# voidstrike/FPSG

Hardware: AMD Instinct MI355X
Metric: episodes/sec (+ Chamfer-kernel HBM GB/s in roofline.hbm), 2048-pt clouds, 224x224 images; episode = fwd + Chamfer + bwd, step = E episodes + all-reduce + Adam (higher is better)
Workload: dtype f32

## Files before the change

### fpsg_amd/_hip.py

```python
from __future__ import annotations

import ctypes
import os
import threading

import torch

_HERE = os.path.dirname(os.path.abspath(__file__))
LIB_PATH = os.environ.get("FPSG_HIP_LIB") or os.path.join(_HERE, "libfpsg_hip.so")

_c_f32p = ctypes.c_void_p
_c_i32p = ctypes.c_void_p
_c_int = ctypes.c_int
_c_stream = ctypes.c_void_p

SIGNATURES = {
    "fpsg_version": [],
    "fpsg_last_error": [],
    "fpsg_chamfer_fwd": [_c_f32p, _c_f32p, _c_int, _c_int, _c_int,
                         _c_f32p, _c_i32p, _c_f32p, _c_i32p, _c_stream],
    "fpsg_chamfer_bwd": [_c_f32p, _c_f32p, _c_i32p, _c_i32p, _c_f32p, _c_f32p,
                         _c_int, _c_int, _c_int, _c_f32p, _c_f32p, _c_stream],
    "fpsg_chamfer_losses": [_c_f32p, _c_f32p, _c_int, _c_int, _c_int, _c_int, ctypes.c_float, ctypes.c_float, _c_f32p,
                            _c_stream],
# ... 62 lines not shown
    "fpsg_bn_act_rows_bwd": [_c_f32p, _c_int, ctypes.POINTER(ctypes.c_int), ctypes.POINTER(ctypes.c_int), _c_int,
                             _c_f32p, _c_f32p, _c_f32p, _c_int, _c_int, ctypes.c_float, _c_f32p, _c_f32p, _c_f32p,
                             _c_f32p, _c_stream],
    "fpsg_bn_workspace_floats": [_c_int, _c_int, _c_int],
    "fpsg_bn_act_fwd": [_c_f32p, _c_f32p, _c_f32p, _c_f32p, _c_f32p, _c_f32p, ctypes.c_float, _c_int, _c_int, _c_int, _c_int,
                        ctypes.c_float, _c_int, ctypes.c_float, _c_f32p, _c_f32p, _c_f32p, _c_f32p, _c_f32p,
                        _c_stream],
    "fpsg_bn_act_bwd": [_c_f32p, _c_f32p, _c_f32p, _c_f32p, _c_int, _c_int, _c_int, _c_int, _c_int,
                        ctypes.c_float, _c_f32p, _c_f32p, _c_f32p, _c_f32p, _c_f32p, _c_f32p, _c_stream],
    "fpsg_bn_act_bwd_coef": [_c_f32p, _c_f32p, _c_f32p, _c_f32p, _c_int, _c_int, _c_int, _c_int, _c_int, ctypes.c_float,
                             _c_f32p, _c_f32p, _c_f32p, _c_f32p, _c_stream],
    "fpsg_bn_act_bwd_parts": [_c_f32p, _c_f32p, _c_f32p, _c_f32p, _c_int, _c_int, _c_int, _c_int, _c_int,
                        ctypes.c_float, _c_f32p, _c_f32p, _c_f32p, _c_f32p, _c_f32p, _c_f32p, _c_f32p, _c_int, _c_stream],
    "fpsg_bn_pool_workspace_floats": [_c_int, _c_int, _c_int, _c_int],
    "fpsg_bn_act_pool_fwd": [_c_f32p, _c_f32p, _c_f32p, _c_f32p, _c_f32p, _c_f32p, ctypes.c_float, _c_int, _c_int, _c_int, _c_int,
                             _c_int, ctypes.c_float, _c_int, ctypes.c_float, _c_f32p, _c_f32p, _c_f32p, _c_f32p,
                             _c_f32p, _c_f32p, _c_int, _c_stream],
    "fpsg_bn_act_pool_bwd": [_c_f32p, _c_f32p, _c_f32p, _c_f32p, _c_int, _c_int, _c_int, _c_int, _c_int, _c_int,
                             ctypes.c_float, _c_f32p, _c_f32p, _c_f32p, _c_f32p, _c_f32p, _c_f32p, _c_stream],
    "fpsg_bn_max_workspace_floats": [_c_int, _c_int, _c_int],
    "fpsg_bn_max_dz_offset": [_c_int, _c_int, _c_int],
    "fpsg_bn_act_max_fwd": [_c_f32p, _c_f32p, _c_f32p, _c_f32p, _c_f32p, _c_f32p, ctypes.c_float, _c_int, _c_int, _c_int, _c_int,
                            ctypes.c_float, _c_int, ctypes.c_float, _c_f32p, _c_i32p, _c_f32p, _c_f32p, _c_f32p,
                            _c_f32p, _c_stream],
    "fpsg_bn_act_max_bwd": [_c_f32p, _c_f32p, _c_f32p, _c_i32p, _c_f32p, _c_int, _c_int, _c_int, _c_int, _c_int,
                            ctypes.c_float, _c_f32p, _c_f32p, _c_f32p, _c_f32p, _c_f32p, _c_f32p, _c_stream],
    "fpsg_max_bwd_prep": [_c_f32p, _c_f32p, _c_f32p, _c_f32p, _c_f32p, _c_f32p, _c_int, _c_int, _c_int, _c_int, _c_f32p, _c_f32p,
                          _c_f32p, _c_f32p, _c_stream],
    "fpsg_max_bwd_dw": [_c_f32p, _c_f32p, _c_f32p, _c_f32p, _c_f32p, _c_int, _c_int, _c_int, _c_f32p, _c_stream],
    "fpsg_max_bwd_gather": [_c_f32p, _c_f32p, _c_i32p, _c_int, _c_int, _c_int, _c_int, _c_f32p, _c_f32p, _c_stream],
    "fpsg_max_bwd_scatter": [_c_f32p, _c_f32p, _c_f32p, _c_f32p, _c_i32p, _c_f32p, _c_int, _c_int, _c_int, _c_int, _c_f32p,
                             _c_stream],
    "fpsg_max_bwd_scatter_workspace_floats": [_c_int, _c_int, _c_int],
    "fpsg_bn_act_max_bwd_coef": [_c_f32p, _c_f32p, _c_f32p, _c_i32p, _c_f32p, _c_int, _c_int, _c_int, _c_int, _c_int,
                                 ctypes.c_float, _c_f32p, _c_f32p, _c_f32p, _c_f32p, _c_stream],
    "fpsg_wino_input_transform": [_c_int, _c_f32p, _c_int, _c_int, _c_int, _c_int, _c_f32p, ctypes.c_long, _c_stream],
    "fpsg_wino_output_transform": [_c_int, _c_f32p, _c_int, _c_int, _c_int, _c_int, _c_f32p, ctypes.c_long, _c_stream],
    "fpsg_wino_stats_parts": [_c_int, _c_int, _c_int, _c_int],
    "fpsg_wino_output_transform_stats": [_c_int, _c_f32p, _c_int, _c_int, _c_int, _c_int, _c_f32p, _c_f32p, _c_f32p,
                                         ctypes.c_long, _c_stream],
    "fpsg_wino_grad_output_transform": [_c_int, _c_f32p, _c_int, _c_int, _c_int, _c_int, _c_f32p, ctypes.c_long, _c_stream],
    "fpsg_wino_grad_transforms": [_c_int, _c_f32p, _c_int, _c_int, _c_int, _c_int, _c_f32p, _c_f32p, ctypes.c_long, _c_stream],
    "fpsg_wino_filter_transform": [_c_int, _c_f32p, _c_int, _c_int, _c_int, _c_f32p, _c_stream],
    "fpsg_wino_output_transform_bwd_stats": [_c_int, _c_f32p, _c_int, _c_int, _c_int, _c_int, _c_f32p, _c_f32p, _c_f32p,
                                             _c_f32p, _c_f32p, ctypes.c_long, _c_stream],
    "fpsg_wino_filter_transform_batch": [ctypes.c_void_p, _c_int, ctypes.c_long, _c_stream],
    "fpsg_wino_filter_grad_transform": [_c_int, _c_f32p, _c_int, _c_int, _c_f32p, _c_stream],
    "fpsg_wino_conv_fused": [_c_f32p, _c_f32p, _c_int, _c_int, _c_int, _c_int, _c_int, _c_f32p, _c_stream],
    "fpsg_wino_input_transform_act": [_c_int, _c_f32p, _c_f32p, _c_f32p, _c_int, _c_int, _c_int, _c_int, _c_f32p, ctypes.c_long,
                                      _c_stream],
    "fpsg_wino_conv_fused_act": [_c_f32p, _c_f32p, _c_f32p, _c_f32p, _c_int, _c_int, _c_int, _c_int, _c_int, _c_f32p,
                                 _c_stream],
    "fpsg_wino_dw_fused_workspace_floats": [_c_int, _c_int, _c_int, _c_int],
    "fpsg_wino_dw_fused": [_c_f32p, _c_f32p, _c_f32p, _c_f32p, _c_int, _c_int, _c_int, _c_int, _c_int, _c_f32p, _c_f32p,
                           _c_stream],
    "fpsg_wino_conv_fused_parts": [_c_int, _c_int, _c_int, _c_int],
    "fpsg_wino_conv_fused_stats": [_c_f32p, _c_f32p, _c_f32p, _c_f32p, _c_int, _c_int, _c_int, _c_int, _c_int, _c_f32p,
                                   _c_f32p, _c_f32p, _c_stream],
    "fpsg_bn_stats": [_c_f32p, _c_f32p, _c_f32p, _c_f32p, _c_f32p, _c_f32p, ctypes.c_float, _c_int, _c_int, _c_int, _c_int,
                      ctypes.c_float, _c_f32p, _c_f32p, _c_f32p, _c_f32p, _c_f32p, _c_int, _c_stream],
    "fpsg_conv_first_dw_workspace_floats": [_c_int, _c_int, _c_int],
    "fpsg_conv_first_parts": [_c_int, _c_int, _c_int],
    "fpsg_conv_first_fwd": [_c_f32p, _c_f32p, _c_int, _c_int, _c_int, _c_int, _c_int, _c_f32p, _c_f32p, _c_f32p, _c_stream],
    "fpsg_conv_first_dw": [_c_f32p, _c_f32p, _c_int, _c_int, _c_int, _c_int, _c_int, _c_f32p, _c_f32p, _c_stream],
    "fpsg_conv_first_dw_fold": [_c_f32p, _c_f32p, _c_f32p, _c_f32p, _c_f32p, _c_f32p, _c_int, _c_int, _c_int, _c_int, _c_int,
                                _c_f32p, _c_f32p, _c_stream],
# ... 96 lines not shown
    "fpsg_points_render": [_c_f32p, ctypes.c_void_p, _c_int, _c_int, _c_f32p, _c_int, _c_int, _c_int, _c_int,
                           ctypes.c_float, ctypes.c_float, ctypes.POINTER(ctypes.c_float), _c_int, ctypes.c_void_p,
                           ctypes.c_void_p, _c_f32p, _c_i32p, _c_f32p, ctypes.c_void_p, ctypes.c_size_t, _c_stream],
    "fpsg_episode_views": [ctypes.c_void_p, _c_int, _c_int, _c_int, _c_i32p, _c_int, _c_i32p, _c_f32p, _c_f32p, _c_int,
                           _c_int, _c_stream],
    "fpsg_point_mesh_workspace_bytes": [_c_int, _c_int, _c_int, _c_int],
    "fpsg_point_mesh_distance": [_c_f32p, _c_int, _c_int, _c_f32p, _c_int, _c_int, _c_i32p, _c_int, _c_int, _c_f32p,
                                 _c_i32p, _c_f32p, _c_f32p, ctypes.c_void_p, ctypes.c_size_t, _c_stream],
    "fpsg_point_normals_workspace_bytes": [_c_int, _c_int, _c_int],
    "fpsg_point_normals": [_c_f32p, _c_int, _c_int, _c_int, _c_int, _c_f32p, _c_f32p, _c_f32p, _c_i32p, ctypes.c_void_p,
                           ctypes.c_size_t, _c_stream],
    "fpsg_point_normals_orient_workspace_bytes": [_c_int, _c_int, _c_int],
    "fpsg_point_normals_orient": [_c_f32p, _c_f32p, _c_i32p, _c_int, _c_int, _c_int, _c_int, _c_f32p, _c_i32p,
                                  ctypes.c_void_p, ctypes.c_size_t, _c_stream],
}
_RESTYPES = {"fpsg_last_error": ctypes.c_char_p, "fpsg_grad_norm_workspace_bytes": ctypes.c_size_t,
"fpsg_chamfer_workspace_bytes": ctypes.c_size_t,
             "fpsg_sinkhorn_workspace_floats": ctypes.c_size_t,
             "fpsg_sinkhorn_grad_workspace_floats": ctypes.c_size_t,
             "fpsg_knn_workspace_floats": ctypes.c_size_t,
             "fpsg_bn_workspace_floats": ctypes.c_size_t, "fpsg_bn_pool_workspace_floats": ctypes.c_size_t, "fpsg_bn_max_workspace_floats": ctypes.c_size_t, "fpsg_bn_max_dz_offset": ctypes.c_size_t, "fpsg_conv_first_dw_workspace_floats": ctypes.c_size_t, "fpsg_emd_workspace_floats": ctypes.c_size_t, "fpsg_emd_exact_workspace_floats": ctypes.c_size_t, "fpsg_emd_cross_workspace_bytes": ctypes.c_size_t, "fpsg_occupancy_grid_workspace_bytes": ctypes.c_size_t, "fpsg_fps_workspace_bytes": ctypes.c_size_t, "fpsg_max_bwd_scatter_workspace_floats": ctypes.c_size_t,
             "fpsg_wino_dw_fused_workspace_floats": ctypes.c_size_t, "fpsg_gemm_split_workspace_floats": ctypes.c_size_t, "fpsg_gemm_split_packed_a_bytes": ctypes.c_size_t, "fpsg_edgeconv_stats_ws_floats": ctypes.c_size_t,
             "fpsg_repulsion_workspace_bytes": ctypes.c_size_t,
             "fpsg_expansion_workspace_bytes": ctypes.c_size_t,
             "fpsg_uniform_workspace_bytes": ctypes.c_size_t,
             "fpsg_swd_workspace_bytes": ctypes.c_size_t,
             "fpsg_mesh_cdf_workspace_bytes": ctypes.c_size_t,
             "fpsg_mesh_render_workspace_bytes": ctypes.c_size_t,
             "fpsg_mesh_render_materials_workspace_bytes": ctypes.c_size_t,
             "fpsg_mesh_render_smooth_workspace_bytes": ctypes.c_size_t,
             "fpsg_points_render_workspace_bytes": ctypes.c_size_t,
             "fpsg_point_mesh_workspace_bytes": ctypes.c_size_t,
             "fpsg_point_normals_workspace_bytes": ctypes.c_size_t,
             "fpsg_point_normals_orient_workspace_bytes": ctypes.c_size_t}

_lib = None
_lock = threading.Lock()


class FpsgHipError(RuntimeError):
    pass


def load() -> ctypes.CDLL:
    global _lib
    if _lib is None:
        with _lock:
            if _lib is None:
                if not os.path.exists(LIB_PATH):
                    raise FpsgHipError(
                        f"{LIB_PATH} not found: build it with `make -C fpsg_amd/csrc` "
                        "(or `python -c 'import __graft_entry__ as g; g.build()'`). "
                        "fpsg_amd has no CPU or PyTorch fallback for its HIP ops.")
                lib = ctypes.CDLL(LIB_PATH)
                for name, argtypes in SIGNATURES.items():
                    fn = getattr(lib, name)
                    fn.argtypes = argtypes
                    fn.restype = _RESTYPES.get(name, ctypes.c_int)
                _lib = lib
    return _lib


def check(rc: int, what: str) -> None:
    if rc != 0:
        msg = load().fpsg_last_error()
        raise FpsgHipError(f"{what} failed (code {rc}): {msg.decode() if msg else ''}")

# ... 22 lines not shown
```

### fpsg_amd/csrc/maxbwd.hip

```cpp
#include "fpsg_common.h"

namespace fpsg {
namespace {

constexpr int kMbThreads = 256;

constexpr int kGatherL = 2048;
constexpr int kGatherNB = 4;

__global__ __launch_bounds__(kMbThreads) void max_bwd_gather_kernel(const float* __restrict__ a, const float* __restrict__ dz,
                                                                   const int32_t* __restrict__ idx, int B, int K, int C,
                                                                   int L, float* __restrict__ S,
                                                                   float* __restrict__ spart ) {
  extern __shared__ __attribute__((aligned(16))) float rows[];
  constexpr int kPre = kGatherNB * kGatherL / 4 / kMbThreads;
  const int k = blockIdx.x;
  const int c = blockIdx.y * kMbThreads + threadIdx.x;
  const bool live = c < C;
  const int L4 = L >> 2;
  const int per_step = kGatherNB * L4;
  float acc = 0.0f;
  auto fetch = [&](int b0, v4f (&pre)[kPre]) {
#pragma unroll
    for (int u = 0; u < kPre; ++u) {
// ... 16 lines not shown
  __syncthreads();
  int step = 0;
  for (int b0 = 0; b0 < B; b0 += kGatherNB, ++step) {
    const float* cur = rows + (size_t)(step & 1) * kGatherNB * L;
    float* nxt = rows + (size_t)((step + 1) & 1) * kGatherNB * L;
    const bool more = b0 + kGatherNB < B;
    if (more) fetch(b0 + kGatherNB, pre);
    if (spart && blockIdx.y == 0) {
      const int w = threadIdx.x >> 6, lane = threadIdx.x & 63;
      if (w < kGatherNB && b0 + w < B) {
        float t = 0.0f;
        for (int l = lane; l < L; l += 64) t += cur[w * L + l];
        t = wave_sum(t);
        if (lane == 0) spart[(size_t)(b0 + w) * K + k] = t;
      }
    }
    if (live) {
      float d[kGatherNB];
      int sel[kGatherNB];
#pragma unroll
      for (int j = 0; j < kGatherNB; ++j) {
        const bool in = b0 + j < B;
        const size_t row = (size_t)(in ? b0 + j : b0) * C + c;
        d[j] = in ? dz[row] : 0.0f;
        sel[j] = in ? idx[row] : 0;
      }
#pragma unroll
      for (int j = 0; j < kGatherNB; ++j) acc = fma_rn(d[j], cur[j * L + sel[j]], acc);
    }
    if (more) park(nxt, pre);
    __syncthreads();
  }
  if (live) S[(size_t)c * K + k] = acc;
}

constexpr int kTL = 128;
constexpr int kCP = 1024;

constexpr int kSortThreadsMb = 512;

__global__ __launch_bounds__(kSortThreadsMb) void max_bwd_sort_kernel(const int32_t* __restrict__ idx, const float* __restrict__ k1,
                                                                     const float* __restrict__ dz, int C, int passes, int tiles,
                                                                     unsigned* __restrict__ skeys ,
                                                                     float* __restrict__ scoef ,
                                                                     int* __restrict__ toff ) {
  __shared__ unsigned keys[kCP];
  constexpr int kMbThreads = kSortThreadsMb;
  const int b = blockIdx.x, tid = threadIdx.x;
  for (int ps = 0; ps < passes; ++ps) {
    const int c0 = ps * kCP;
    for (int e = tid; e < kCP; e += kMbThreads) {
      const int c = c0 + e;
      keys[e] = c < C ? (((unsigned)idx[(size_t)b * C + c] << 16) | (unsigned)e) : 0xffffffffu;
    }
    __syncthreads();
    for (int span = 2; span <= kCP; span <<= 1) {
      for (int j = span >> 1; j > 0; j >>= 1) {
        for (int e = tid; e < kCP; e += kMbThreads) {
          const int p = e ^ j;
          if (p > e) {
            const unsigned x = keys[e], y = keys[p];
            const bool up = (e & span) == 0;
            if ((x > y) == up) { keys[e] = y; keys[p] = x; }
          }
        }
        __syncthreads();
// ... 73 lines not shown
        if (lane < K) D[ql[u] * ld + lane] = fma_rn(cf[u], w0[u], D[ql[u] * ld + lane]);
        if (lane + 64 < K) D[ql[u] * ld + lane + 64] = fma_rn(cf[u], w1[u], D[ql[u] * ld + lane + 64]);
      }
    }
  }
  __syncthreads();
  const bool pair_ok = (L & 1) == 0;
  for (int k0 = wave; k0 < K; k0 += 8 * (kMbThreads / 64)) {
    v2f r[8];
    const int l = 2 * lane;
#pragma unroll
    for (int u = 0; u < 8; ++u) {
      const int k = k0 + u * (kMbThreads / 64);
      r[u] = (v2f){0.0f, 0.0f};
      if (k < K) {
        const float* row = da + ((size_t)b * K + k) * L + l0;
        if (pair_ok && l0 + l + 1 < L) r[u] = *reinterpret_cast<const v2f*>(row + l);
        else { if (l0 + l < L) r[u][0] = row[l]; if (l0 + l + 1 < L) r[u][1] = row[l + 1]; }
      }
    }
#pragma unroll
    for (int u = 0; u < 8; ++u) {
      const int k = k0 + u * (kMbThreads / 64);
      if (k >= K) continue;
      const float vk = v[k];
      float* row = da + ((size_t)b * K + k) * L + l0;
      const v2f o = {r[u][0] + (vk + D[l * ld + k]), r[u][1] + (vk + D[(l + 1) * ld + k])};
      if (pair_ok && l0 + l + 1 < L) *reinterpret_cast<v2f*>(row + l) = o;
      else { if (l0 + l < L) row[l] = o[0]; if (l0 + l + 1 < L) row[l + 1] = o[1]; }
    }
  }
}

__global__ __launch_bounds__(kMbThreads) void max_bwd_prep_kernel(const float* __restrict__ W, const float* __restrict__ coef,
                                                                 const float* __restrict__ pb, const float* __restrict__ mean,
                                                                 const float* __restrict__ dz, const float* __restrict__ spart,
                                                                 int B, int K, int C, float count, float* __restrict__ Wk,
                                                                 float* __restrict__ u, float* __restrict__ dpb,
                                                                 float* __restrict__ s_out) {
  const long e = (long)blockIdx.x * kMbThreads + threadIdx.x;
  if (e >= (long)C * K) return;
  const int c = (int)(e / K), k = (int)(e - (long)c * K);
  const float k1 = coef[c], k2 = coef[C + c], k3 = coef[2 * C + c];
  Wk[e] = k2 * W[e];
  if (k == 0) {
    const float b = pb ? pb[c] : 0.0f;
    u[c] = fma_rn(k2, b, k3);
    if (dpb) {
      float sum = 0.0f;
      int n = 0;
      for (; n + 8 <= B; n += 8) {
        float t[8];
#pragma unroll
        for (int j = 0; j < 8; ++j) t[j] = dz[(size_t)(n + j) * C + c];
#pragma unroll
        for (int j = 0; j < 8; ++j) sum += t[j];
      }
      for (; n < B; ++n) sum += dz[(size_t)n * C + c];
      dpb[c] = fma_rn(k1, sum, fma_rn(k2, mean[c], k3) * count);
    }
  }
  if (c == 0 && spart) {
    float sk = 0.0f;
    int n = 0;
    for (; n + 8 <= B; n += 8) {
      float t[8];
#pragma unroll
      for (int j = 0; j < 8; ++j) t[j] = spart[(size_t)(n + j) * K + k];
#pragma unroll
      for (int j = 0; j < 8; ++j) sk += t[j];
    }
    for (; n < B; ++n) sk += spart[(size_t)n * K + k];
    s_out[k] = sk;
  }
}

__global__ __launch_bounds__(kMbThreads) void max_bwd_dw_kernel(const float* __restrict__ S, const float* __restrict__ WG,
                                                               const float* __restrict__ coef, const float* __restrict__ pb,
                                                               const float* __restrict__ spart, int B, int K, int C,
                                                               float* __restrict__ dw) {
  const long e = (long)blockIdx.x * kMbThreads + threadIdx.x;
  if (e >= (long)C * K) return;
  const int c = (int)(e / K), k = (int)(e - (long)c * K);
  const float k1 = coef[c], k2 = coef[C + c], k3 = coef[2 * C + c];
  float r = k1 * S[e];
  if (WG) {
    const float sk = spart[k];
    const float b = pb ? pb[c] : 0.0f;
    r = fma_rn(k2, fma_rn(b, sk, WG[e]), r);
    r = fma_rn(k3, sk, r);
  }
  dw[e] = r;
}

}
}

extern "C" int fpsg_max_bwd_gather(const float* a, const float* dz, const int32_t* idx, int B, int K, int C, int L,
                                   float* S, float* spart, fpsg_stream_t stream) {
  using namespace fpsg;
  FPSG_REQUIRE(B > 0 && K > 0 && C > 0 && L > 0, FPSG_E_SHAPE, "fpsg_max_bwd_gather: B,K,C,L must be positive (got %d,%d,%d,%d)",
               B, K, C, L);
  FPSG_REQUIRE(K <= 65535 && (C + 255) / 256 <= 65535, FPSG_E_LIMIT, "fpsg_max_bwd_gather: C=%d or K=%d beyond the grid", C, K);
  FPSG_REQUIRE_PTR(a); FPSG_REQUIRE_PTR(dz); FPSG_REQUIRE_PTR(idx); FPSG_REQUIRE_PTR(S);
  FPSG_REQUIRE(L % 4 == 0 && L <= kGatherL, FPSG_E_LIMIT, "fpsg_max_bwd_gather: L=%d must be a multiple of 4, at most %d", L, kGatherL);
  FPSG_REQUIRE((reinterpret_cast<uintptr_t>(a) & 15) == 0, FPSG_E_ALIGN, "fpsg_max_bwd_gather: a must be 16-byte aligned");
  dim3 grid(K, (C + kMbThreads - 1) / kMbThreads);
  const size_t lds_bytes = (size_t)2 * kGatherNB * L * sizeof(float);
  FPSG_REQUIRE(!misaligned4(spart), FPSG_E_ALIGN, "fpsg_max_bwd_gather: spart not 4-byte aligned");
  hipLaunchKernelGGL(max_bwd_gather_kernel, grid, dim3(kMbThreads), lds_bytes, static_cast<hipStream_t>(stream), a, dz, idx, B, K, C,
                     L, S, spart);
  return launch_status("fpsg_max_bwd_gather");
}

extern "C" size_t fpsg_max_bwd_scatter_workspace_floats(int B, int C, int L) {
  if (B <= 0 || C <= 0 || L <= 0) return 0;
  const size_t passes = (C + fpsg::kCP - 1) / fpsg::kCP, tiles = (L + fpsg::kTL - 1) / fpsg::kTL;
  return (size_t)B * passes * (2 * fpsg::kCP + tiles + 1);
}

extern "C" int fpsg_max_bwd_scatter(float* da, const float* W, const float* k1, const float* dz, const int32_t* idx,
                                    const float* v, int B, int K, int C, int L, float* ws, fpsg_stream_t stream) {
  using namespace fpsg;
  FPSG_REQUIRE(B > 0 && K > 0 && C > 0 && L > 0, FPSG_E_SHAPE, "fpsg_max_bwd_scatter: B,K,C,L must be positive (got %d,%d,%d,%d)",
               B, K, C, L);
  FPSG_REQUIRE(K <= 128, FPSG_E_LIMIT, "fpsg_max_bwd_scatter: K=%d beyond 128 input channels (two per lane)", K);
  FPSG_REQUIRE(L <= 65535 - kTL && B <= 65535, FPSG_E_LIMIT,
               "fpsg_max_bwd_scatter: B=%d or L=%d beyond the 16-bit point field of the sort keys / the grid", B, L);
  FPSG_REQUIRE_PTR(da); FPSG_REQUIRE_PTR(W); FPSG_REQUIRE_PTR(k1); FPSG_REQUIRE_PTR(dz); FPSG_REQUIRE_PTR(idx); FPSG_REQUIRE_PTR(v);
  FPSG_REQUIRE_PTR(ws);
  hipStream_t s = static_cast<hipStream_t>(stream);
  const int passes = (C + kCP - 1) / kCP, tiles = (L + kTL - 1) / kTL;
  unsigned* skeys = reinterpret_cast<unsigned*>(ws);
  float* scoef = ws + (size_t)B * passes * kCP;
  int* toff = reinterpret_cast<int*>(ws + (size_t)2 * B * passes * kCP);
  hipLaunchKernelGGL(max_bwd_sort_kernel, dim3(B), dim3(kSortThreadsMb), 0, s, idx, k1, dz, C, passes, tiles, skeys, scoef, toff);
  int rc = launch_status("fpsg_max_bwd_scatter(sort)");
  if (rc) return rc;
  const size_t lds_bytes = ((size_t)kTL * (K + 1) + 2 * kCP) * sizeof(float);
  if (lds_bytes > 65536) {
    hipError_t e = hipFuncSetAttribute(reinterpret_cast<const void*>(max_bwd_scatter_kernel),
                                       hipFuncAttributeMaxDynamicSharedMemorySize, (int)lds_bytes);
    if (e != hipSuccess) { set_error("fpsg_max_bwd_scatter: %s", hipGetErrorString(e)); return (int)e; }
  }
  dim3 grid((L + kTL - 1) / kTL, B);
  hipLaunchKernelGGL(max_bwd_scatter_kernel, grid, dim3(kMbThreads), lds_bytes, s, da, W, skeys, scoef, toff, v, K, C, L, passes, tiles);
  return launch_status("fpsg_max_bwd_scatter");
}

extern "C" int fpsg_max_bwd_prep(const float* W, const float* coef, const float* pre_bias, const float* mean, const float* dz,
                                 const float* spart, int B, int K, int C, int L, float* Wk, float* u, float* dpre_bias,
                                 float* s, fpsg_stream_t stream) {
  using namespace fpsg;
  FPSG_REQUIRE(B > 0 && K > 0 && C > 0 && L > 0, FPSG_E_SHAPE, "fpsg_max_bwd_prep: B,K,C,L must be positive (got %d,%d,%d,%d)", B, K, C, L);
  FPSG_REQUIRE_PTR(W); FPSG_REQUIRE_PTR(coef); FPSG_REQUIRE_PTR(mean); FPSG_REQUIRE_PTR(dz); FPSG_REQUIRE_PTR(Wk); FPSG_REQUIRE_PTR(u);
  FPSG_REQUIRE(!misaligned4(pre_bias) && !misaligned4(dpre_bias) && !misaligned4(spart) && !misaligned4(s), FPSG_E_ALIGN,
               "fpsg_max_bwd_prep: pre_bias / dpre_bias / spart / s not 4-byte aligned");
  FPSG_REQUIRE((spart == nullptr) == (s == nullptr), FPSG_E_NULL, "fpsg_max_bwd_prep: spart and s go together");
  const long n = (long)C * K;
  hipLaunchKernelGGL(max_bwd_prep_kernel, dim3((unsigned)((n + kMbThreads - 1) / kMbThreads)), dim3(kMbThreads), 0,
                     static_cast<hipStream_t>(stream), W, coef, pre_bias, mean, dz, spart, B, K, C, (float)((double)B * (double)L), Wk,
                     u, dpre_bias, s);
  return launch_status("fpsg_max_bwd_prep");
}

extern "C" int fpsg_max_bwd_dw(const float* S, const float* WG, const float* coef, const float* pre_bias, const float* s,
                               int B, int K, int C, float* dw, fpsg_stream_t stream) {
  using namespace fpsg;
  FPSG_REQUIRE(B > 0 && K > 0 && C > 0, FPSG_E_SHAPE, "fpsg_max_bwd_dw: B,K,C must be positive (got %d,%d,%d)", B, K, C);
  FPSG_REQUIRE_PTR(S); FPSG_REQUIRE_PTR(coef); FPSG_REQUIRE_PTR(dw);
  FPSG_REQUIRE(!misaligned4(WG) && !misaligned4(pre_bias) && !misaligned4(s), FPSG_E_ALIGN, "fpsg_max_bwd_dw: not 4-byte aligned");
  FPSG_REQUIRE(WG == nullptr || s != nullptr, FPSG_E_NULL, "fpsg_max_bwd_dw: s missing");
  const long n = (long)C * K;
  hipLaunchKernelGGL(max_bwd_dw_kernel, dim3((unsigned)((n + kMbThreads - 1) / kMbThreads)), dim3(kMbThreads), 0,
                     static_cast<hipStream_t>(stream), S, WG, coef, pre_bias, s, B, K, C, dw);
  return launch_status("fpsg_max_bwd_dw");
}
```

### fpsg_amd/fused_bn.py

```python
from __future__ import annotations

import os

import torch
import torch.nn as nn
import torch.nn.functional as F

from .bn_counters import count_batch
from . import _hip, conv_first, winograd

_ACT_CODES = {None: 0, "none": 0, "relu": 1, "leaky": 2}
_MIN_ROW = 64
ROWS_SEGMENT_MAX = 16384


def fused_enabled() -> bool:
    return os.environ.get("FPSG_FUSED_BN", "1") != "0"


def _parse_act(act):
    if isinstance(act, tuple):
        return _ACT_CODES[act[0]], float(act[1])
    return _ACT_CODES[act], 0.0

# ... 198 lines not shown
        x, chan, idx, pre_bias = ctx.saved_tensors
        N, C, L, training, act_code, slope, has_w, has_b = ctx.cfg
        want_dpb = pre_bias is not None and ctx.needs_input_grad[9]
        lib = _hip.load()
        dev = x.device
        gout = gout.contiguous()
        dx = torch.empty_like(x)
        dgamma = torch.empty((C,), dtype=torch.float32, device=dev)
        dbeta = torch.empty((C,), dtype=torch.float32, device=dev)
        dpb = torch.empty((C,), dtype=torch.float32, device=dev) if want_dpb else None
        coef = torch.empty((3, C), dtype=torch.float32, device=dev)
        ws = torch.empty((lib.fpsg_bn_max_workspace_floats(N, C, L),), dtype=torch.float32, device=dev)
        with torch.cuda.device(dev):
            rc = lib.fpsg_bn_act_max_bwd(_hip.ptr(x), _hip.ptr(pre_bias) if pre_bias is not None else None,
                                         _hip.ptr(gout), _hip.ptr(idx), _hip.ptr(chan), N, C, L,
                                         1 if training else 0, act_code, float(slope), _hip.ptr(dx),
                                         _hip.ptr(dgamma), _hip.ptr(dbeta), _hip.ptr(dpb) if want_dpb else None,
                                         _hip.ptr(coef), _hip.ptr(ws), _hip.stream_of(x))
        _hip.check(rc, "fpsg_bn_act_max_bwd")
        return dx, (dgamma if has_w else None), (dbeta if has_b else None), None, None, None, None, None, None, dpb, None


def W_is_plain(conv) -> bool:
    return conv.weight.is_contiguous() and conv.weight.dim() == 3 and conv.weight.shape[2] == 1


_MAX_ALGEBRA_MIN_POINTS = 16384


def max_bwd_algebra_enabled() -> bool:
    return os.environ.get("FPSG_MAX_BWD_ALGEBRA", "1") != "0"


class _ConvBNActMax(torch.autograd.Function):

    @staticmethod
    def forward(ctx, a, weight, conv_bias, gamma, beta, running_mean, running_var, training, eps, act_code, slope, momentum):
        B, K, L = a.shape
        C = weight.shape[0]
        lib = _hip.load()
        dev = a.device
        W = weight.reshape(C, K)
        x = torch.bmm(W.unsqueeze(0).expand(B, -1, -1), a)
        out = torch.empty((B, C), dtype=torch.float32, device=dev)
        idx = torch.empty((B, C), dtype=torch.int32, device=dev)
        chan, mode = _chan_and_mode(training, gamma, beta, running_mean, running_var, eps, C, dev)
        ws = torch.empty((lib.fpsg_bn_max_workspace_floats(B, C, L),), dtype=torch.float32, device=dev)
        opt = lambda t: _hip.ptr(t) if t is not None else None
        with torch.cuda.device(dev):
            rc = lib.fpsg_bn_act_max_fwd(_hip.ptr(x), opt(conv_bias), opt(gamma), opt(beta), opt(running_mean),
                                         opt(running_var), float(momentum), B, C, L, mode, float(eps),
                                         act_code, float(slope), _hip.ptr(out), _hip.ptr(idx), _hip.ptr(chan), None,
                                         None, _hip.ptr(ws), _hip.stream_of(a))
        _hip.check(rc, "fpsg_bn_act_max_fwd")
        ctx.save_for_backward(a, weight, x, chan, idx, conv_bias)
        ctx.cfg = (B, K, C, L, bool(training), act_code, slope, gamma is not None, beta is not None)
        return out

    @staticmethod
    def backward(ctx, gout):
        a, weight, x, chan, idx, pb = ctx.saved_tensors
        B, K, C, L, training, act_code, slope, has_g, has_b = ctx.cfg
        lib = _hip.load()
        dev = a.device
        gout = gout.contiguous()
        W = weight.reshape(C, K)
        dgamma = torch.empty((C,), dtype=torch.float32, device=dev)
        dbeta = torch.empty((C,), dtype=torch.float32, device=dev)
        coef = torch.empty((3, C), dtype=torch.float32, device=dev)
        ws = torch.empty((lib.fpsg_bn_max_workspace_floats(B, C, L),), dtype=torch.float32, device=dev)
        st = _hip.stream_of(a)
        with torch.cuda.device(dev):
            _hip.check(lib.fpsg_bn_act_max_bwd_coef(_hip.ptr(x), _hip.ptr(pb) if pb is not None else None, _hip.ptr(gout),
                                                    _hip.ptr(idx), _hip.ptr(chan), B, C, L, 1 if training else 0, act_code,
                                                    float(slope), _hip.ptr(dgamma), _hip.ptr(dbeta), _hip.ptr(coef),
                                                    _hip.ptr(ws), st), "fpsg_bn_act_max_bwd_coef")
            off = lib.fpsg_bn_max_dz_offset(B, C, L)
            dz = ws[off: off + B * C].view(B, C)
            opt = lambda t: _hip.ptr(t) if t is not None else None
            da = dw = dpb = None
            want_dpb = pb is not None and ctx.needs_input_grad[2]
            Wk = torch.empty((C, K), dtype=torch.float32, device=dev)
            u = torch.empty((C,), dtype=torch.float32, device=dev)
            if want_dpb:
                dpb = torch.empty((C,), dtype=torch.float32, device=dev)
            spart = s = S = None
            if ctx.needs_input_grad[1]:
                S = torch.empty((C, K), dtype=torch.float32, device=dev)
                if training:
                    spart = torch.empty((B, K), dtype=torch.float32, device=dev)
                    s = torch.empty((K,), dtype=torch.float32, device=dev)
                _hip.check(lib.fpsg_max_bwd_gather(_hip.ptr(a), _hip.ptr(dz), _hip.ptr(idx), B, K, C, L, _hip.ptr(S), opt(spart),
                                                   st), "fpsg_max_bwd_gather")
            _hip.check(lib.fpsg_max_bwd_prep(_hip.ptr(W), _hip.ptr(coef), opt(pb), _hip.ptr(chan[2]), _hip.ptr(dz), opt(spart),
                                             B, K, C, L, _hip.ptr(Wk), _hip.ptr(u), opt(dpb), opt(s), st), "fpsg_max_bwd_prep")
            if ctx.needs_input_grad[1]:
                WG = None
                if training:
                    G = torch.bmm(a, a.transpose(1, 2)).sum(0)
                    WG = W @ G
                dw = torch.empty((C, K), dtype=torch.float32, device=dev)
                _hip.check(lib.fpsg_max_bwd_dw(_hip.ptr(S), opt(WG), _hip.ptr(coef), opt(pb), opt(s), B, K, C, _hip.ptr(dw),
                                               st), "fpsg_max_bwd_dw")
                dw = dw.reshape(weight.shape)
            if ctx.needs_input_grad[0]:
                if training:
                    M = W.t() @ Wk
                    v = torch.mv(W.t(), u)
                    da = torch.bmm(M.unsqueeze(0).expand(B, -1, -1), a)
                else:
                    v = torch.zeros((K,), dtype=torch.float32, device=dev)
                    da = torch.zeros_like(a)
                sws = torch.empty((lib.fpsg_max_bwd_scatter_workspace_floats(B, C, L),), dtype=torch.float32, device=dev)
                _hip.check(lib.fpsg_max_bwd_scatter(_hip.ptr(da), _hip.ptr(W), _hip.ptr(coef), _hip.ptr(dz), _hip.ptr(idx),
                                                    _hip.ptr(v), B, K, C, L, _hip.ptr(sws), st), "fpsg_max_bwd_scatter")
        return (da, dw, dpb, dgamma if has_g else None, dbeta if has_b else None, None, None, None, None, None, None, None)


def _eligible(x: torch.Tensor) -> bool:
    if not (x.is_cuda and x.dtype == torch.float32 and x.dim() >= 3 and fused_enabled()):
        return False
    row = x.numel() // max(x.shape[0] * x.shape[1], 1)
    return row >= _MIN_ROW and row % 4 == 0 and x.shape[1] <= 65535


def _plain_act(y, act_code, slope):
    if act_code == 1:
        return F.relu(y)
    if act_code == 2:
        return F.leaky_relu(y, slope)
    return y


def batch_norm_act(x, weight, bias, running_mean, running_var, training, momentum, eps, act=None,
                   return_stats: bool = False, pre_bias=None):
    act_code, slope = _parse_act(act)
    if _eligible(x):
        xc = x.contiguous()
        update = training and not return_stats and running_mean is not None
        m = (0.1 if momentum is None else float(momentum)) if update else -1.0
        y, bmean, bvar = _BNAct.apply(xc, weight, bias, running_mean, running_var, bool(training), eps,
                                      act_code, slope, bool(training and return_stats), pre_bias, m)
        return (y, bmean, bvar) if return_stats else y
    if pre_bias is not None:
        x = x + pre_bias.view(1, -1, *([1] * (x.dim() - 2)))
    if return_stats:
        C = x.shape[1]
        mean = torch.zeros(C, dtype=x.dtype, device=x.device)
# ... 149 lines not shown
```

### include/fpsg_hip.h

```cpp
#ifndef FPSG_HIP_H
#define FPSG_HIP_H

#include <stddef.h>
#include <stdint.h>

#ifdef __cplusplus
extern "C" {
#endif

typedef void* fpsg_stream_t;

#define FPSG_ABI_VERSION 1

#define FPSG_E_NULL   (-1)
#define FPSG_E_SHAPE  (-2)
#define FPSG_E_ALIGN  (-3)
#define FPSG_E_LIMIT  (-4)

int         fpsg_version(void);
const char* fpsg_last_error(void);

int fpsg_chamfer_fwd(const float* xyz1, const float* xyz2, int B, int N, int M,
                     float* dist1, int32_t* idx1, float* dist2, int32_t* idx2,
                     fpsg_stream_t stream);
// ... 218 lines not shown
int fpsg_bn_act_pool_fwd(const float* x, const float* pre_bias, const float* gamma, const float* beta,
                         float* running_mean, float* running_var, float momentum, int N, int C, int H, int W,
                         int training, float eps, int act, float slope, float* y_pooled, float* chan,
                         float* batch_mean, float* batch_var_unbiased, float* ws, const float* parts, int n_parts,
                         fpsg_stream_t stream);
int fpsg_bn_act_pool_bwd(const float* x, const float* pre_bias, const float* dy_pooled, const float* chan,
                         int N, int C, int H, int W, int training, int act, float slope, float* dx,
                         float* dgamma, float* dbeta, float* dpre_bias, float* coef, float* ws,
                         fpsg_stream_t stream);

size_t fpsg_bn_max_workspace_floats(int N, int C, int L);
size_t fpsg_bn_max_dz_offset(int N, int C, int L);
int fpsg_bn_act_max_fwd(const float* x, const float* pre_bias, const float* gamma, const float* beta,
                        float* running_mean, float* running_var, float momentum, int N, int C, int L, int training,
                        float eps, int act, float slope, float* out, int32_t* idx, float* chan, float* batch_mean,
                        float* batch_var_unbiased, float* ws, fpsg_stream_t stream);
int fpsg_bn_act_max_bwd(const float* x, const float* pre_bias, const float* gout, const int32_t* idx,
                        const float* chan, int N, int C, int L, int training, int act, float slope, float* dx,
                        float* dgamma, float* dbeta, float* dpre_bias, float* coef, float* ws, fpsg_stream_t stream);
int fpsg_bn_act_max_bwd_coef(const float* x, const float* pre_bias, const float* gout, const int32_t* idx,
                             const float* chan, int N, int C, int L, int training, int act, float slope,
                             float* dgamma, float* dbeta, float* coef, float* ws, fpsg_stream_t stream);

int fpsg_max_bwd_gather(const float* a, const float* dz, const int32_t* idx, int B, int K, int C, int L, float* S,
                        float* spart , fpsg_stream_t stream);
int fpsg_max_bwd_prep(const float* W, const float* coef, const float* pre_bias, const float* mean, const float* dz,
                      const float* spart, int B, int K, int C, int L, float* Wk, float* u, float* dpre_bias, float* s,
                      fpsg_stream_t stream);
int fpsg_max_bwd_dw(const float* S, const float* WG, const float* coef, const float* pre_bias, const float* s, int B,
                    int K, int C, float* dw, fpsg_stream_t stream);
size_t fpsg_max_bwd_scatter_workspace_floats(int B, int C, int L);
int fpsg_max_bwd_scatter(float* da, const float* W, const float* k1, const float* dz, const int32_t* idx, const float* v,
                         int B, int K, int C, int L, float* ws, fpsg_stream_t stream);


int fpsg_wino_input_transform(int m, const float* x, int N, int C, int H, int W, float* V, long ldp,
                              fpsg_stream_t stream);
int fpsg_wino_output_transform(int m, const float* M, int N, int K, int H, int W, float* y, long ldp,
                               fpsg_stream_t stream);
int fpsg_wino_stats_parts(int m, int N, int H, int W);
int fpsg_wino_output_transform_stats(int m, const float* M, int N, int K, int H, int W, float* y, const float* bias,
                                     float* parts, long ldp, fpsg_stream_t stream);
int fpsg_wino_output_transform_bwd_stats(int m, const float* M, int N, int K, int H, int W, float* y,
                                         const float* xpre, const float* pre_bias, const float* chan,
                                         float* parts, long ldp, fpsg_stream_t stream);
int fpsg_wino_grad_output_transform(int m, const float* dy, int N, int K, int H, int W, float* dM, long ldp,
                                    fpsg_stream_t stream);
int fpsg_wino_grad_transforms(int m, const float* dy, int N, int K, int H, int W, float* V, float* dM, long ldp,
                              fpsg_stream_t stream);
int fpsg_wino_filter_transform(int m, const float* w, int K, int C, int flip_transpose, float* U,
                               fpsg_stream_t stream);
int fpsg_wino_filter_transform_batch(const int64_t* jobs, int n_jobs, long total_blocks, fpsg_stream_t stream);
int fpsg_wino_filter_grad_transform(int m, const float* dU, int K, int C, float* dw, fpsg_stream_t stream);

size_t fpsg_gemm_split_workspace_floats(int batch, int M, int N, int K, int transB, int variant);
int fpsg_gemm_split(const float* A, const float* B, float* C, int batch, int M, int N, int K, int lda, int ldb, int ldc,
                    long sA, long sB, long sC, int transB, int variant, float* ws, size_t ws_floats,
                    fpsg_stream_t stream);

size_t fpsg_gemm_split_packed_a_bytes(int batch, int M, int K, int variant);
int fpsg_gemm_split_pack_a(const float* A, int batch, int M, int K, int lda, long sA, int variant, void* Ap,
                           fpsg_stream_t stream);
int fpsg_gemm_split_nn_packed(const void* Ap, const float* B, float* C, int batch, int M, int N, int K, int ldb, int ldc,
                              long sB, long sC, int variant, fpsg_stream_t stream);

int fpsg_gemm_split_nn_persistent(const void* Ap, const float* B, float* C, int batch, int M, int N, int K, int ldb, int ldc,
// ... 145 lines not shown
```

Baseline: 46.23.

## Restructure max-pool backward gather into column-gather plus column-sum, add 512-thread scatter

The max-pool backward gather is split into two kernels. The first stages a few input rows in LDS, reads each row once and gathers the argmax-selected columns into a lent workspace (also computing row sums). The second reduces those columns against dz over the batch. This replaces the old per-(k,C) gather, which re-read rows, at the cost of an extra workspace buffer and its write/read traffic. A 512-thread scatter variant prefetches da rows into registers and batches eight W reads per wave, both enabled by default through an environment flag.

Result: no change. 46.43 (median of 4 runs) (+0.4%).

```diff
diff --git a/fpsg_amd/_hip.py b/fpsg_amd/_hip.py
--- a/fpsg_amd/_hip.py
+++ b/fpsg_amd/_hip.py
@@ -118,6 +118,10 @@
     "fpsg_max_bwd_scatter": [_c_f32p, _c_f32p, _c_f32p, _c_f32p, _c_i32p, _c_f32p, _c_int, _c_int, _c_int, _c_int, _c_f32p,
                              _c_stream],
     "fpsg_max_bwd_scatter_workspace_floats": [_c_int, _c_int, _c_int],
+    "fpsg_max_bwd_gather_workspace_floats": [_c_int, _c_int, _c_int, _c_int],
+    "fpsg_max_bwd_gather_lend_workspace": [_c_f32p, ctypes.c_size_t],
+    "fpsg_max_bwd_scatter_streamed": [_c_f32p, _c_f32p, _c_f32p, _c_f32p, _c_i32p, _c_f32p, _c_int, _c_int, _c_int, _c_int,
+                                      _c_f32p, _c_stream],
     "fpsg_bn_act_max_bwd_coef": [_c_f32p, _c_f32p, _c_f32p, _c_i32p, _c_f32p, _c_int, _c_int, _c_int, _c_int, _c_int,
                                  ctypes.c_float, _c_f32p, _c_f32p, _c_f32p, _c_f32p, _c_stream],
     "fpsg_wino_input_transform": [_c_int, _c_f32p, _c_int, _c_int, _c_int, _c_int, _c_f32p, ctypes.c_long, _c_stream],
@@ -280,7 +284,8 @@
              "fpsg_points_render_workspace_bytes": ctypes.c_size_t,
              "fpsg_point_mesh_workspace_bytes": ctypes.c_size_t,
              "fpsg_point_normals_workspace_bytes": ctypes.c_size_t,
-             "fpsg_point_normals_orient_workspace_bytes": ctypes.c_size_t}
+             "fpsg_point_normals_orient_workspace_bytes": ctypes.c_size_t,
+             "fpsg_max_bwd_gather_workspace_floats": ctypes.c_size_t}
 
 _lib = None
 _lock = threading.Lock()
diff --git a/fpsg_amd/csrc/maxbwd.hip b/fpsg_amd/csrc/maxbwd.hip
--- a/fpsg_amd/csrc/maxbwd.hip
+++ b/fpsg_amd/csrc/maxbwd.hip
@@ -72,6 +72,81 @@
     __syncthreads();
   }
   if (live) S[(size_t)c * K + k] = acc;
+}
+
+constexpr int kColRows = 8;
+constexpr int kColThreads = 512;
+constexpr int kColPad = 4;
+
+__global__ __launch_bounds__(kColThreads) void max_bwd_columns_kernel(const float* __restrict__ a, const int32_t* __restrict__ idx,
+                                                                     int K, int C, int L,
+                                                                     float* __restrict__ g ,
+                                                                     float* __restrict__ spart ) {
+  extern __shared__ __attribute__((aligned(16))) float rows[];
+  constexpr int kPre = 8;
+  const int k0 = blockIdx.x * kColRows, b = blockIdx.y;
+  const int nrows = min(kColRows, K - k0);
+  const int L4 = L >> 2, ld = L + kColPad;
+  const int n4 = nrows * L4;
+  const v4f* src = reinterpret_cast<const v4f*>(a + ((size_t)b * K + k0) * L);
+  for (int e0 = threadIdx.x; e0 < n4; e0 += kPre * kColThreads) {
+    v4f pre[kPre];
+#pragma unroll
+    for (int u = 0; u < kPre; ++u) {
+      const int e = e0 + u * kColThreads;
+      pre[u] = (v4f){0.0f, 0.0f, 0.0f, 0.0f};
+      if (e < n4) pre[u] = src[e];
+    }
+#pragma unroll
+    for (int u = 0; u < kPre; ++u) {
+      const int e = e0 + u * kColThreads;
+      const int j = e / L4, q = e - j * L4;
+      if (e < n4) *reinterpret_cast<v4f*>(rows + j * ld + 4 * q) = pre[u];
+    }
+  }
+  __syncthreads();
+  if (spart) {
+    const int w = threadIdx.x >> 6, lane = threadIdx.x & 63;
+    if (w < nrows) {
+      float t = 0.0f;
+      for (int l = lane; l < L; l += 64) t += rows[w * ld + l];
+      t = wave_sum(t);
+      if (lane == 0) spart[(size_t)b * K + k0 + w] = t;
+    }
+  }
+  const int q = threadIdx.x & 1;
+  float* out = g + ((size_t)b * gridDim.x + blockIdx.x) * C * kColRows + 4 * q;
+#pragma unroll 4
+  for (int c = threadIdx.x >> 1; c < C; c += kColThreads / 2) {
+    const int sel = idx[(size_t)b * C + c];
+    v4f col;
+#pragma unroll
+    for (int i = 0; i < 4; ++i) col[i] = 4 * q + i < nrows ? rows[(4 * q + i) * ld + sel] : 0.0f;
+    *reinterpret_cast<v4f*>(out + (size_t)c * kColRows) = col;
+  }
+}
+
+__global__ __launch_bounds__(kMbThreads) void max_bwd_colsum_kernel(const float* __restrict__ g, const float* __restrict__ dz,
+                                                                   int B, int K, int C, float* __restrict__ S) {
+  const long f = (long)blockIdx.x * kMbThreads + threadIdx.x;
+  const long per_group = (long)C * kColRows;
+  const long n = per_group * ((K + kColRows - 1) / kColRows);
+  if (f >= n) return;
+  const int grp = (int)(f / per_group);
+  const int rem = (int)(f - grp * per_group);
+  const int c = rem / kColRows, k = grp * kColRows + (rem - c * kColRows);
+  if (k >= K) return;
+  float acc = 0.0f;
+  int b = 0;
+  for (; b + 8 <= B; b += 8) {
+    float x[8], d[8];
+#pragma unroll
+    for (int j = 0; j < 8; ++j) { x[j] = g[(size_t)(b + j) * n + f]; d[j] = dz[(size_t)(b + j) * C + c]; }
+#pragma unroll
+    for (int j = 0; j < 8; ++j) acc = fma_rn(d[j], x[j], acc);
+  }
+  for (; b < B; ++b) acc = fma_rn(dz[(size_t)b * C + c], g[(size_t)b * n + f], acc);
+  S[(size_t)c * K + k] = acc;
 }
 
 constexpr int kTL = 128;
@@ -211,6 +286,90 @@
   }
 }
 
+constexpr int kStThreads = 512;
+
+__global__ __launch_bounds__(kStThreads) void max_bwd_scatter_streamed_kernel(float* __restrict__ da, const float* __restrict__ W,
+                                                                           const unsigned* __restrict__ skeys,
+                                                                           const float* __restrict__ scoef,
+                                                                           const int* __restrict__ toff,
+                                                                           const float* __restrict__ v, int K, int C, int L,
+                                                                           int passes, int tiles) {
+  constexpr int kThreads = kStThreads, kWaves = kThreads / 64;
+  constexpr int kRows = 128 / kWaves;
+  extern __shared__ __attribute__((aligned(16))) float lds[];
+  const int ld = K + 1;
+  float* D = lds;
+  unsigned* ek = reinterpret_cast<unsigned*>(lds + kTL * ld);
+  float* ec = lds + kTL * ld + kCP;
+  const int b = blockIdx.y;
+  const int l0 = blockIdx.x * kTL;
+  const int tid = threadIdx.x, lane = tid & 63, wave = tid >> 6;
+  const bool pair_ok = (L & 1) == 0;
+  const int l = 2 * lane;
+  v2f r[kRows];
+#pragma unroll
+  for (int u = 0; u < kRows; ++u) {
+    const int k = wave + u * kWaves;
+    r[u] = (v2f){0.0f, 0.0f};
+    if (k < K) {
+      const float* row = da + ((size_t)b * K + k) * L + l0;
+      if (pair_ok && l0 + l + 1 < L) r[u] = *reinterpret_cast<const v2f*>(row + l);
+      else { if (l0 + l < L) r[u][0] = row[l]; if (l0 + l + 1 < L) r[u][1] = row[l + 1]; }
+    }
+  }
+  for (int e = tid; e < kTL * ld; e += kThreads) D[e] = 0.0f;
+  for (int ps = 0; ps < passes; ++ps) {
+    const size_t base = ((size_t)b * passes + ps) * kCP;
+    const int* tf = toff + ((size_t)b * passes + ps) * (tiles + 1) + blockIdx.x;
+    const int first = tf[0], n = tf[1] - first;
+    const int c0 = ps * kCP;
+    __syncthreads();
+    for (int e = tid; e < n; e += kThreads) { ek[e] = skeys[base + first + e]; ec[e] = scoef[base + first + e]; }
+    __syncthreads();
+    for (int q0 = 0; q0 < n; q0 += 64) {
+      const bool in = q0 + lane < n;
+      const unsigned key = in ? ek[q0 + lane] : 0u;
+      const float coef = in ? ec[q0 + lane] : 0.0f;
+      unsigned long long mine = __ballot(in && ((((int)(key >> 16) - l0) & (kWaves - 1)) == wave));
+      while (mine) {
+        int ql[8];
+        float cf[8], w0[8], w1[8];
+#pragma unroll
+        for (int u = 0; u < 8; ++u) {
+          ql[u] = -1; cf[u] = 0.0f; w0[u] = 0.0f; w1[u] = 0.0f;
+          if (mine) {
+            const int i = __ffsll((long long)mine) - 1;
+            mine &= mine - 1;
+            const unsigned ki = (unsigned)__builtin_amdgcn_readlane((int)key, i);
+            const int c = c0 + (int)(ki & 0xffffu);
+            ql[u] = (int)(ki >> 16) - l0;
+            cf[u] = __int_as_float(__builtin_amdgcn_readlane(__float_as_int(coef), i));
+            w0[u] = lane < K ? W[(size_t)c * K + lane] : 0.0f;
+            w1[u] = lane + 64 < K ? W[(size_t)c * K + lane + 64] : 0.0f;
+          }
+        }
+#pragma unroll
+        for (int u = 0; u < 8; ++u) {
+          if (ql[u] < 0) continue;
+          if (lane < K) D[ql[u] * ld + lane] = fma_rn(cf[u], w0[u], D[ql[u] * ld + lane]);
+          if (lane + 64 < K) D[ql[u] * ld + lane + 64] = fma_rn(cf[u], w1[u], D[ql[u] * ld + lane + 64]);
+        }
+      }
+    }
+  }
+  __syncthreads();
+#pragma unroll
+  for (int u = 0; u < kRows; ++u) {
+    const int k = wave + u * kWaves;
+    if (k >= K) continue;
+    const float vk = v[k];
+    float* row = da + ((size_t)b * K + k) * L + l0;
+    const v2f o = {r[u][0] + (vk + D[l * ld + k]), r[u][1] + (vk + D[(l + 1) * ld + k])};
+    if (pair_ok && l0 + l + 1 < L) *reinterpret_cast<v2f*>(row + l) = o;
+    else { if (l0 + l < L) row[l] = o[0]; if (l0 + l + 1 < L) row[l + 1] = o[1]; }
+  }
+}
+
 __global__ __launch_bounds__(kMbThreads) void max_bwd_prep_kernel(const float* __restrict__ W, const float* __restrict__ coef,
                                                                  const float* __restrict__ pb, const float* __restrict__ mean,
                                                                  const float* __restrict__ dz, const float* __restrict__ spart,
@@ -275,9 +434,34 @@
 }
 }
 
+namespace fpsg {
+namespace {
+thread_local float* t_gather_ws = nullptr;
+thread_local size_t t_gather_ws_floats = 0;
+}
+}
+
+extern "C" size_t fpsg_max_bwd_gather_workspace_floats(int B, int K, int C, int L) {
+  if (B <= 0 || K <= 0 || C <= 0 || L <= 0) return 0;
+  return (size_t)B * ((K + fpsg::kColRows - 1) / fpsg::kColRows) * C * fpsg::kColRows;
+}
+
+extern "C" int fpsg_max_bwd_gather_lend_workspace(float* ws, size_t floats) {
+  using namespace fpsg;
+  FPSG_REQUIRE((ws == nullptr) == (floats == 0), FPSG_E_NULL, "fpsg_max_bwd_gather_lend_workspace: ws and floats go together");
+  FPSG_REQUIRE((reinterpret_cast<uintptr_t>(ws) & 15) == 0, FPSG_E_ALIGN, "fpsg_max_bwd_gather_lend_workspace: ws must be 16-byte aligned");
+  t_gather_ws = ws;
+  t_gather_ws_floats = floats;
+  return 0;
+}
+
 extern "C" int fpsg_max_bwd_gather(const float* a, const float* dz, const int32_t* idx, int B, int K, int C, int L,
                                    float* S, float* spart, fpsg_stream_t stream) {
   using namespace fpsg;
+  float* const lent = t_gather_ws;
+  const size_t lent_floats = t_gather_ws_floats;
+  t_gather_ws = nullptr;
+  t_gather_ws_floats = 0;
   FPSG_REQUIRE(B > 0 && K > 0 && C > 0 && L > 0, FPSG_E_SHAPE, "fpsg_max_bwd_gather: B,K,C,L must be positive (got %d,%d,%d,%d)",
                B, K, C, L);
   FPSG_REQUIRE(K <= 65535 && (C + 255) / 256 <= 65535, FPSG_E_LIMIT, "fpsg_max_bwd_gather: C=%d or K=%d beyond the grid", C, K);
@@ -287,6 +471,27 @@
   dim3 grid(K, (C + kMbThreads - 1) / kMbThreads);
   const size_t lds_bytes = (size_t)2 * kGatherNB * L * sizeof(float);
   FPSG_REQUIRE(!misaligned4(spart), FPSG_E_ALIGN, "fpsg_max_bwd_gather: spart not 4-byte aligned");
+  if (lent) {
+    FPSG_REQUIRE(lent_floats >= fpsg_max_bwd_gather_workspace_floats(B, K, C, L), FPSG_E_SHAPE,
+                 "fpsg_max_bwd_gather: the lent workspace holds %zu floats, %zu needed", lent_floats,
+                 fpsg_max_bwd_gather_workspace_floats(B, K, C, L));
+    FPSG_REQUIRE(B <= 65535, FPSG_E_LIMIT, "fpsg_max_bwd_gather: B=%d beyond the grid", B);
+    hipStream_t s = static_cast<hipStream_t>(stream);
+    const size_t col_lds = (size_t)kColRows * (L + kColPad) * sizeof(float);
+    if (col_lds > 65536) {
+      hipError_t e = hipFuncSetAttribute(reinterpret_cast<const void*>(max_bwd_columns_kernel),
+                                         hipFuncAttributeMaxDynamicSharedMemorySize, (int)col_lds);
+      if (e != hipSuccess) { set_error("fpsg_max_bwd_gather: %s", hipGetErrorString(e)); return (int)e; }
+    }
+    hipLaunchKernelGGL(max_bwd_columns_kernel, dim3((K + kColRows - 1) / kColRows, B), dim3(kColThreads), col_lds, s, a, idx, K, C, L,
+                       lent, spart);
+    int rc = launch_status("fpsg_max_bwd_gather(columns)");
+    if (rc) return rc;
+    const long n = (long)C * kColRows * ((K + kColRows - 1) / kColRows);
+    hipLaunchKernelGGL(max_bwd_colsum_kernel, dim3((unsigned)((n + kMbThreads - 1) / kMbThreads)), dim3(kMbThreads), 0, s, lent, dz, B,
+                       K, C, S);
+    return launch_status("fpsg_max_bwd_gather(column sums)");
+  }
   hipLaunchKernelGGL(max_bwd_gather_kernel, grid, dim3(kMbThreads), lds_bytes, static_cast<hipStream_t>(stream), a, dz, idx, B, K, C,
                      L, S, spart);
   return launch_status("fpsg_max_bwd_gather");
@@ -298,9 +503,11 @@
   return (size_t)B * passes * (2 * fpsg::kCP + tiles + 1);
 }
 
-extern "C" int fpsg_max_bwd_scatter(float* da, const float* W, const float* k1, const float* dz, const int32_t* idx,
-                                    const float* v, int B, int K, int C, int L, float* ws, fpsg_stream_t stream) {
-  using namespace fpsg;
+namespace fpsg {
+namespace {
+template <bool kStreamed>
+int max_bwd_scatter_launch(float* da, const float* W, const float* k1, const float* dz, const int32_t* idx, const float* v,
+                           int B, int K, int C, int L, float* ws, fpsg_stream_t stream) {
   FPSG_REQUIRE(B > 0 && K > 0 && C > 0 && L > 0, FPSG_E_SHAPE, "fpsg_max_bwd_scatter: B,K,C,L must be positive (got %d,%d,%d,%d)",
                B, K, C, L);
   FPSG_REQUIRE(K <= 128, FPSG_E_LIMIT, "fpsg_max_bwd_scatter: K=%d beyond 128 input channels (two per lane)", K);
@@ -317,14 +524,28 @@
   int rc = launch_status("fpsg_max_bwd_scatter(sort)");
   if (rc) return rc;
   const size_t lds_bytes = ((size_t)kTL * (K + 1) + 2 * kCP) * sizeof(float);
+  const auto kernel = kStreamed ? max_bwd_scatter_streamed_kernel : max_bwd_scatter_kernel;
+  const int threads = kStreamed ? kStThreads : kMbThreads;
   if (lds_bytes > 65536) {
-    hipError_t e = hipFuncSetAttribute(reinterpret_cast<const void*>(max_bwd_scatter_kernel),
-                                       hipFuncAttributeMaxDynamicSharedMemorySize, (int)lds_bytes);
+    hipError_t e = hipFuncSetAttribute(reinterpret_cast<const void*>(kernel), hipFuncAttributeMaxDynamicSharedMemorySize,
+                                       (int)lds_bytes);
     if (e != hipSuccess) { set_error("fpsg_max_bwd_scatter: %s", hipGetErrorString(e)); return (int)e; }
   }
   dim3 grid((L + kTL - 1) / kTL, B);
-  hipLaunchKernelGGL(max_bwd_scatter_kernel, grid, dim3(kMbThreads), lds_bytes, s, da, W, skeys, scoef, toff, v, K, C, L, passes, tiles);
+  hipLaunchKernelGGL(kernel, grid, dim3(threads), lds_bytes, s, da, W, skeys, scoef, toff, v, K, C, L, passes, tiles);
   return launch_status("fpsg_max_bwd_scatter");
+}
+}
+}
+
+extern "C" int fpsg_max_bwd_scatter(float* da, const float* W, const float* k1, const float* dz, const int32_t* idx,
+                                    const float* v, int B, int K, int C, int L, float* ws, fpsg_stream_t stream) {
+  return fpsg::max_bwd_scatter_launch<false>(da, W, k1, dz, idx, v, B, K, C, L, ws, stream);
+}
+
+extern "C" int fpsg_max_bwd_scatter_streamed(float* da, const float* W, const float* k1, const float* dz, const int32_t* idx,
+                                             const float* v, int B, int K, int C, int L, float* ws, fpsg_stream_t stream) {
+  return fpsg::max_bwd_scatter_launch<true>(da, W, k1, dz, idx, v, B, K, C, L, ws, stream);
 }
 
 extern "C" int fpsg_max_bwd_prep(const float* W, const float* coef, const float* pre_bias, const float* mean, const float* dz,
diff --git a/fpsg_amd/fused_bn.py b/fpsg_amd/fused_bn.py
--- a/fpsg_amd/fused_bn.py
+++ b/fpsg_amd/fused_bn.py
@@ -254,6 +254,10 @@
     return os.environ.get("FPSG_MAX_BWD_ALGEBRA", "1") != "0"
 
 
+def max_bwd_one_pass_enabled() -> bool:
+    return os.environ.get("FPSG_MAX_BWD_ONE_PASS", "1") != "0"
+
+
 class _ConvBNActMax(torch.autograd.Function):
 
     @staticmethod
@@ -292,6 +296,7 @@
         coef = torch.empty((3, C), dtype=torch.float32, device=dev)
         ws = torch.empty((lib.fpsg_bn_max_workspace_floats(B, C, L),), dtype=torch.float32, device=dev)
         st = _hip.stream_of(a)
+        one_pass = max_bwd_one_pass_enabled()
         with torch.cuda.device(dev):
             _hip.check(lib.fpsg_bn_act_max_bwd_coef(_hip.ptr(x), _hip.ptr(pb) if pb is not None else None, _hip.ptr(gout),
                                                     _hip.ptr(idx), _hip.ptr(chan), B, C, L, 1 if training else 0, act_code,
@@ -312,6 +317,10 @@
                 if training:
                     spart = torch.empty((B, K), dtype=torch.float32, device=dev)
                     s = torch.empty((K,), dtype=torch.float32, device=dev)
+                if one_pass:
+                    n = lib.fpsg_max_bwd_gather_workspace_floats(B, K, C, L)
+                    gws = torch.empty((n,), dtype=torch.float32, device=dev)
+                    _hip.check(lib.fpsg_max_bwd_gather_lend_workspace(_hip.ptr(gws), n), "fpsg_max_bwd_gather_lend_workspace")
                 _hip.check(lib.fpsg_max_bwd_gather(_hip.ptr(a), _hip.ptr(dz), _hip.ptr(idx), B, K, C, L, _hip.ptr(S), opt(spart),
                                                    st), "fpsg_max_bwd_gather")
             _hip.check(lib.fpsg_max_bwd_prep(_hip.ptr(W), _hip.ptr(coef), opt(pb), _hip.ptr(chan[2]), _hip.ptr(dz), opt(spart),
@@ -334,8 +343,9 @@
                     v = torch.zeros((K,), dtype=torch.float32, device=dev)
                     da = torch.zeros_like(a)
                 sws = torch.empty((lib.fpsg_max_bwd_scatter_workspace_floats(B, C, L),), dtype=torch.float32, device=dev)
-                _hip.check(lib.fpsg_max_bwd_scatter(_hip.ptr(da), _hip.ptr(W), _hip.ptr(coef), _hip.ptr(dz), _hip.ptr(idx),
-                                                    _hip.ptr(v), B, K, C, L, _hip.ptr(sws), st), "fpsg_max_bwd_scatter")
+                scatter = lib.fpsg_max_bwd_scatter_streamed if one_pass else lib.fpsg_max_bwd_scatter
+                _hip.check(scatter(_hip.ptr(da), _hip.ptr(W), _hip.ptr(coef), _hip.ptr(dz), _hip.ptr(idx), _hip.ptr(v), B, K, C, L,
+                                   _hip.ptr(sws), st), "fpsg_max_bwd_scatter")
         return (da, dw, dpb, dgamma if has_g else None, dbeta if has_b else None, None, None, None, None, None, None, None)
 
 
diff --git a/include/fpsg_hip.h b/include/fpsg_hip.h
--- a/include/fpsg_hip.h
+++ b/include/fpsg_hip.h
@@ -274,6 +274,10 @@
 size_t fpsg_max_bwd_scatter_workspace_floats(int B, int C, int L);
 int fpsg_max_bwd_scatter(float* da, const float* W, const float* k1, const float* dz, const int32_t* idx, const float* v,
                          int B, int K, int C, int L, float* ws, fpsg_stream_t stream);
+size_t fpsg_max_bwd_gather_workspace_floats(int B, int K, int C, int L);
+int fpsg_max_bwd_gather_lend_workspace(float* ws, size_t floats);
+int fpsg_max_bwd_scatter_streamed(float* da, const float* W, const float* k1, const float* dz, const int32_t* idx,
+                                  const float* v, int B, int K, int C, int L, float* ws, fpsg_stream_t stream);
 
 
 int fpsg_wino_input_transform(int m, const float* x, int N, int C, int H, int W, float* V, long ldp,
```
